# shicaiwei123/ICCV2025-GDL

Measured on AMD Instinct MI355X. Metric: audio-visual samples/sec, CREMA-D DGL train step (whole job), higher is better.
Workload: dtype bf16; 1 GPU; CREMA-D DGL (main_dgl.py, ConcatFusion_DGL) ResNet18 a+v, spec 1x257x188 + frames 3x3x224x224, alpha=4, SGD lr 2e-3 mom .9 wd 1e-4, clip 40; per_gpu_batch=64, global_batch=64, parallelism=dp1, buckets=none

## Files before the change

iccv2025-gdl_amd/csrc/conv_wgrad.hip:

```cpp
#include <stdlib.h>

#include "common.h"
#include "gather.h"
#include "prof.h"

#include <hip/hip_ext.h>

namespace gdl {

struct WgradArgs {
    const void* dy;
    const void* x;
    float* partial;
    const GatherEntry* table;
    int C, K, RS, M;
    int nsplit, chunk;
    int tiles_k, tiles_c;
    unsigned dy_bytes, x_bytes;
    int delta[9];
    int split;
    int delta_hi[9];
#ifdef GDL_TIMING
    unsigned long long* dbg;
#endif
// ... 142 lines not shown
#ifdef GDL_TIMING
    unsigned long long t_entry = __builtin_amdgcn_s_memtime(), t_wait = 0, t_comp = 0, t_issue = 0, t_a, t_b;
#endif
    if (nst > 0) load_stage(0);
#ifdef GDL_TIMING
    unsigned long long t_first = __builtin_amdgcn_s_memtime();
#endif
    for (int st = 0; st < nst; ++st) {
        const int buf = st & 1;
#ifdef GDL_TIMING
        t_a = __builtin_amdgcn_s_memtime();
#endif
        asm volatile("s_waitcnt vmcnt(0)" ::: "memory");
        __builtin_amdgcn_s_barrier();
        asm volatile("" ::: "memory");
#ifdef GDL_TIMING
        t_b = __builtin_amdgcn_s_memtime();
        t_wait += t_b - t_a;
#endif
        if (st + 1 < nst) load_stage(buf ^ 1);
#ifdef GDL_TIMING
        t_a = __builtin_amdgcn_s_memtime();
        t_issue += t_a - t_b;
#endif
        const unsigned Ks = smem_base + buf * STAGE;
        const unsigned Cs = Ks + WG_BP * PK;
        if (sizeof(T) == 2) {
#pragma unroll
            for (int ks = 0; ks < WG_BP / 32; ++ks) {
                uint2 alo[FK], ahi[FK], blo[FC], bhi[FC];
#pragma unroll
                for (int h = 0; h < 2; ++h) {
                    const int row = ks * 32 + g * 8 + h * 4 + (li >> 2);
#pragma unroll
                    for (int i = 0; i < FK; ++i) {
                        const int chb = (wk * WTK + i * 16 + (li & 3) * 4) * 2;
                        const int addr = row * PK + ((((chb >> 5) ^ wg_swz<PK>(row)) << 5) | (chb & 31));
                        if (h == 0)
                            alo[i] = lds_tr16_asm(Ks + addr);
                        else
                            ahi[i] = lds_tr16_asm(Ks + addr);
                    }
#pragma unroll
                    for (int jj = 0; jj < FC; ++jj) {
                        const int chb = (wc * WTC + jj * 16 + (li & 3) * 4) * 2;
                        const int addr = row * PC + ((((chb >> 5) ^ wg_swz<PC>(row)) << 5) | (chb & 31));
                        if (h == 0)
                            blo[jj] = lds_tr16_asm(Cs + addr);
                        else
                            bhi[jj] = lds_tr16_asm(Cs + addr);
                    }
                }
                wg_lds_wait();
#pragma unroll
                for (int i = 0; i < FK; ++i) {
                    const uint4 fa = make_uint4(alo[i].x, alo[i].y, ahi[i].x, ahi[i].y);
#pragma unroll
                    for (int jj = 0; jj < FC; ++jj) {
                        const uint4 fb = make_uint4(blo[jj].x, blo[jj].y, bhi[jj].x, bhi[jj].y);
                        acc[i][jj] = __builtin_amdgcn_mfma_f32_16x16x32_bf16(__builtin_bit_cast(bf16x8_t, fa),
                                                                           __builtin_bit_cast(bf16x8_t, fb), acc[i][jj], 0,
                                                                           0, 0);
                    }
                }
            }
        } else {
#pragma unroll 4
            for (int ks = 0; ks < WG_BP / 4; ++ks) {
                const int row = ks * 4 + g;
                float fa[FK], fb[FC];
#pragma unroll
                for (int i = 0; i < FK; ++i) {
                    const int chb = (wk * WTK + i * 16 + li) * 4;
                    fa[i] = lds_read_f32_asm(Ks + row * PK + ((((chb >> 5) ^ wg_swz<PK>(row)) << 5) | (chb & 31)));
                }
#pragma unroll
                for (int jj = 0; jj < FC; ++jj) {
                    const int chb = (wc * WTC + jj * 16 + li) * 4;
                    fb[jj] = lds_read_f32_asm(Cs + row * PC + ((((chb >> 5) ^ wg_swz<PC>(row)) << 5) | (chb & 31)));
                }
                wg_lds_wait();
#pragma unroll
                for (int i = 0; i < FK; ++i)
#pragma unroll
                    for (int jj = 0; jj < FC; ++jj)
                        acc[i][jj] = __builtin_amdgcn_mfma_f32_16x16x4f32(fa[i], fb[jj], acc[i][jj], 0, 0, 0);
            }
        }
    }
#ifdef GDL_TIMING
    unsigned long long t_loop_end = __builtin_amdgcn_s_memtime();
    t_comp = (t_loop_end - t_first) - t_wait - t_issue;
#endif
    float* part = a.partial + (size_t)slice * a.K * RS * a.C;
#pragma unroll
    for (int i = 0; i < FK; ++i)
#pragma unroll
        for (int jj = 0; jj < FC; ++jj) {
            const int c = c0 + wc * WTC + jj * 16 + li;
#pragma unroll
            for (int e = 0; e < 4; ++e) {
                const int k = k0 + wk * WTK + i * 16 + g * 4 + e;
                part[((size_t)k * RS + tap) * a.C + c] = acc[i][jj][e];
            }
        }
#ifdef GDL_TIMING
    if (a.dbg && tid == 0) {
        unsigned long long* d = a.dbg + (size_t)blockIdx.x * 8;
        d[0] = t_entry;
        d[1] = t_first - t_entry;
        d[2] = t_wait;
        d[3] = t_issue;
        d[4] = t_comp;
        d[5] = __builtin_amdgcn_s_memtime() - t_loop_end;
        d[6] = nst;
    }
#endif
}

template <int LANES>
__global__ __launch_bounds__(256) void wgrad_reduce_kernel(const float* __restrict__ partial, float* __restrict__ out,
                                                           int nsplit, int K, int RS, int C, int Cout) {
    constexpr int OUTS = 256 / LANES;
    __shared__ float red[LANES][OUTS];
    const size_t total = (size_t)K * RS * C;
    const int o = threadIdx.x % OUTS, l = threadIdx.x / OUTS;
    const size_t i = blockIdx.x * (size_t)OUTS + o;
    float s = 0.f;
    if (i < total)
        for (int sp = l; sp < nsplit; sp += LANES) s += partial[(size_t)sp * total + i];
    if (LANES > 1) {
        red[l][o] = s;
        __syncthreads();
        if (l == 0) {
            s = red[0][o];
#pragma unroll
            for (int j = 1; j < LANES; ++j) s += red[j][o];
        }
    }
    if (l == 0 && i < total) {
        const int c = (int)(i % C);
        const size_t t = i / C;
        const int rs = (int)(t % RS);
        const int k = (int)(t / RS);
        if (c < Cout) out[((size_t)k * Cout + c) * RS + rs] = s;
    }
}

bool conv_wgrad9_enabled();
bool conv_wgrad9_ok(int dtype, int W, int C, int K, int R, int S, int stride, int pad);
size_t conv_wgrad9_ws_bytes(int M, int C, int K);
int conv_wgrad9(const void* dy, const void* x, float* dw, const void* table, int N, int H, int W, int C, int K, void* ws,
                size_t ws_bytes, hipStream_t st);

struct WgradPlan {
    int tk, tc, nsplit, chunk;
};

static WgradPlan plan_wgrad(int M, int C, int K, int RS, bool gemm = false) {
    WgradPlan p;
    p.tk = (K % 128 == 0) ? 128 : 64;
    p.tc = (C % 128 == 0) ? 128 : 64;
    const int tiles = (K / p.tk) * (C / p.tc) * RS;
    static int forced = -1;
    if (forced < 0) {
        const char* e = tune_env("GDL_WGRAD_BLOCKS");
        forced = e ? atoi(e) : 0;
    }
    static int forced_gemm = -1;
    if (forced_gemm < 0) {
        const char* e = tune_env("GDL_WGRAD_GEMM_BLOCKS");
        forced_gemm = e ? atoi(e) : 0;
    }
    const int target = (gemm && forced_gemm > 0) ? forced_gemm : forced > 0 ? forced : (gemm ? 416 : 128);
    int ns = (target + tiles - 1) / tiles;
    const int max_ns = (M + 2 * WG_BP - 1) / (2 * WG_BP);
    if (ns > max_ns) ns = max_ns;
    if (ns < 1) ns = 1;
    int chunk = (M + ns - 1) / ns;
    chunk = (chunk + WG_BP - 1) / WG_BP * WG_BP;
    p.nsplit = (M + chunk - 1) / chunk;
    p.chunk = chunk;
    return p;
}

size_t conv_wgrad_ws_bytes(int M, int C, int K, int RS) {
    const WgradPlan p = plan_wgrad(M, C, K, RS, RS == 1);
    size_t b = (size_t)p.nsplit * K * RS * C * sizeof(float);
    if (RS == 9 && conv_wgrad9_enabled()) {
        const size_t b9 = conv_wgrad9_ws_bytes(M, C, K);
        if (b9 > b) b = b9;
    }
    return b;
}

template <typename T, int TK, int TC>
static int launch_wg(WgradArgs& a, hipStream_t st) {
    constexpr int BYTES = 2 * WG_BP * (TK + TC) * (int)sizeof(T);
    auto kfn = conv_wgrad_kernel<T, TK, TC>;
    static DevOnce attr_set;
    if (!attr_set) {
        hipError_t e = hipFuncSetAttribute((const void*)kfn, hipFuncAttributeMaxDynamicSharedMemorySize, BYTES);
        if (e != hipSuccess) return check_hip(e, "hipFuncSetAttribute(conv_wgrad)");
        attr_set = true;
    }
    const int per_slice = a.RS * a.tiles_k * a.tiles_c;
    const int grid = xcd_grid(a.nsplit * per_slice);
    static char pname[96] = "";
    if (!pname[0]) snprintf(pname, sizeof(pname), "gdl::conv_wgrad_kernel<%s, %d, %d>", prof_tname<T>(), TK, TC);
    ProfScope prof(pname, PROF_MFMA, st, 2.0 * (double)a.M * a.K * a.C * a.RS, true,
                   (double)a.dy_bytes + (double)a.x_bytes + 4.0 * (double)a.K * a.C * a.RS);
    hipExtLaunchKernelGGL(kfn, dim3(grid), dim3(256), BYTES, st, prof.e0(), prof.e1(), 0, a);
    GDL_CHECK_LAUNCH("conv_wgrad_kernel");
    return GDL_OK;
}

int conv_wgrad(int dtype, const void* dy, const void* x, float* dw, const void* table, int N, int H, int W, int C, int K,
               int R, int S, int stride, int pad, int Cout, void* ws, size_t ws_bytes, hipStream_t st) {
    GDL_REQUIRE(dtype == GDL_BF16 || dtype == GDL_F32, "wgrad: bad dtype %d", dtype);
    GDL_REQUIRE(table, "wgrad: gather table is null (build it with gdl_conv_build_table)");
    GDL_REQUIRE(C % 64 == 0 && K % 64 == 0, "wgrad: C=%d K=%d must be multiples of 64", C, K);
    if (Cout == C && conv_wgrad9_ok(dtype, W, C, K, R, S, stride, pad))
        return conv_wgrad9(dy, x, dw, table, N, H, W, C, K, ws, ws_bytes, st);
    GatherGeom g;
    int rc = gather_geom(GATHER_FWD, dtype, N, H, W, C, K, R, S, stride, pad, &g);
    if (rc) return rc;
    const int esz = dtype == GDL_BF16 ? 2 : 4;
    WgradArgs a{};
#ifdef GDL_TIMING
    a.dbg = g_timing_buf;
#endif
    a.dy = dy;
    a.x = x;
    a.table = (const GatherEntry*)table;
    a.C = C;
    a.K = K;
    a.RS = R * S;
    a.M = g.rows;
    for (int t = 0; t < 9; ++t) a.delta[t] = g.delta[t];
    GDL_REQUIRE(a.M < (1 << 24), "wgrad: M exceeds 2^24");
    GDL_REQUIRE((size_t)a.M * K * esz < (1UL << 31), "wgrad: dy exceeds 2 GiB");
    a.dy_bytes = (unsigned)((size_t)a.M * K * esz);
    a.x_bytes = (unsigned)((size_t)N * H * W * C * esz);
    const WgradPlan p = plan_wgrad(a.M, C, K, R * S, R == 1 && S == 1 && stride == 1);
    a.nsplit = p.nsplit;
    a.chunk = p.chunk;
    a.tiles_k = K / p.tk;
    a.tiles_c = C / p.tc;
    const size_t need = (size_t)p.nsplit * K * R * S * C * sizeof(float);
    if (ws_bytes < need || !ws) {
        set_error("wgrad: workspace %zu < %zu bytes", ws_bytes, need);
        return GDL_ERR_WORKSPACE;
    }
    a.partial = (float*)ws;
    if (dtype == GDL_BF16) {
        if (p.tk == 128 && p.tc == 128)
            rc = launch_wg<bf16, 128, 128>(a, st);
        else if (p.tk == 128)
            rc = launch_wg<bf16, 128, 64>(a, st);
        else if (p.tc == 128)
            rc = launch_wg<bf16, 64, 128>(a, st);
        else
            rc = launch_wg<bf16, 64, 64>(a, st);
    } else {
        if (p.tk == 128 && p.tc == 128)
            rc = launch_wg<float, 128, 128>(a, st);
        else if (p.tk == 128)
            rc = launch_wg<float, 128, 64>(a, st);
        else if (p.tc == 128)
            rc = launch_wg<float, 64, 128>(a, st);
        else
            rc = launch_wg<float, 64, 64>(a, st);
    }
    if (rc) return rc;
    const size_t total = (size_t)K * R * S * C;
#ifdef GDL_EXPERIMENT
    if (experiment_mask2() & 1) return GDL_OK;
#endif
    ProfScope prof(p.nsplit >= 64 ? "gdl::wgrad_reduce_kernel<16>" : (p.nsplit > 8 ? "gdl::wgrad_reduce_kernel<4>" : "gdl::wgrad_reduce_kernel<1>"),
                   PROF_HBM, st, (double)total * 4.0 * (p.nsplit + 1));
    if (p.nsplit >= 64)
        hipLaunchKernelGGL(wgrad_reduce_kernel<16>, dim3((unsigned)((total + 15) / 16)), dim3(256), 0, st, a.partial, dw,
                           p.nsplit, K, R * S, C, Cout);
    else if (p.nsplit > 8)
        hipLaunchKernelGGL(wgrad_reduce_kernel<4>, dim3((unsigned)((total + 63) / 64)), dim3(256), 0, st, a.partial, dw,
                           p.nsplit, K, R * S, C, Cout);
    else
        hipLaunchKernelGGL(wgrad_reduce_kernel<1>, dim3((unsigned)((total + 255) / 256)), dim3(256), 0, st, a.partial, dw,
                           p.nsplit, K, R * S, C, Cout);
    GDL_CHECK_LAUNCH("wgrad_reduce_kernel");
    return GDL_OK;
}

__global__ __launch_bounds__(256) void stem_wgrad_reduce_kernel(const float* __restrict__ partial, float* __restrict__ out,
                                                                int nsplit, int Cin) {
    __shared__ float4 red[16][16];
    constexpr int TILE4 = 64 * 4 * 64 / 4;
    const int o = threadIdx.x & 15, l = threadIdx.x >> 4;
    const int idx4 = blockIdx.x * 16 + o;
    const float4* p = (const float4*)partial + idx4;
    float4 s = make_float4(0.f, 0.f, 0.f, 0.f);
    int sp = l;
    for (; sp + 48 < nsplit; sp += 64) {
        const float4 v0 = p[(size_t)sp * TILE4], v1 = p[(size_t)(sp + 16) * TILE4];
        const float4 v2 = p[(size_t)(sp + 32) * TILE4], v3 = p[(size_t)(sp + 48) * TILE4];
        s.x += v0.x, s.y += v0.y, s.z += v0.z, s.w += v0.w;
        s.x += v1.x, s.y += v1.y, s.z += v1.z, s.w += v1.w;
        s.x += v2.x, s.y += v2.y, s.z += v2.z, s.w += v2.w;
        s.x += v3.x, s.y += v3.y, s.z += v3.z, s.w += v3.w;
    }
    for (; sp < nsplit; sp += 16) {
        const float4 v0 = p[(size_t)sp * TILE4];
        s.x += v0.x, s.y += v0.y, s.z += v0.z, s.w += v0.w;
    }
    red[l][o] = s;
    __syncthreads();
    if (l != 0) return;
#pragma unroll
    for (int jj = 1; jj < 16; ++jj) {
        const float4 v = red[jj][o];
        s.x += v.x, s.y += v.y, s.z += v.z, s.w += v.w;
    }
    const int q = idx4 & 15, tap = (idx4 >> 4) & 3, k = idx4 >> 6;
    const int r = 2 * tap + (q >> 3), px = q & 7;
    if (r < 7 && px < 7) {
        const float v[4] = {s.x, s.y, s.z, s.w};
        for (int c = 0; c < Cin; ++c) out[((k * Cin + c) * 7 + r) * 7 + px] = v[c];
    }
}

struct StemRowsArgs {
    const void* dy;
    const void* xp;
    float* partial;
    int P, Q, Hp, Wp, nseg;
    int stages, chunk, nsplit;
    unsigned dy_bytes, x_bytes;
};
constexpr int SR_PITCH = 1088, SR_XBYTES = 9 * 1024, SR_STAGE = 8192 + SR_XBYTES;
template <int OFF>
__device__ __forceinline__ uint2 sr_tr(unsigned addr) {
    uint2 v;
    asm volatile("ds_read_b64_tr_b16 %0, %1 offset:%2" : "=v"(v) : "v"(addr), "n"(OFF));
    return v;
}
template <int N>
__device__ __forceinline__ void sr_wait() {
    __builtin_amdgcn_sched_barrier(0);
    asm volatile("s_waitcnt lgkmcnt(%0)" ::"n"(N) : "memory");
    __builtin_amdgcn_sched_barrier(0);
}
__global__ __launch_bounds__(256) void stem_wgrad_rows_kernel(StemRowsArgs a) {
    extern __shared__ __attribute__((aligned(16))) unsigned char smem[];
    const int tid = threadIdx.x, lane = tid & 63, wave = __builtin_amdgcn_readfirstlane(tid >> 6);
    const int g = lane >> 4, li = lane & 15;
    const int slice = blockIdx.x;
    const int s_begin = slice * a.chunk, s_end = min(a.stages, s_begin + a.chunk);
    const int nst = s_end - s_begin;
    const unsigned smem_base = (unsigned)(uintptr_t)(const __attribute__((address_space(3))) unsigned char*)smem;
    const __amdgpu_buffer_rsrc_t rdy = __builtin_amdgcn_make_buffer_rsrc((void*)a.dy, 0, a.dy_bytes, 0x00020000);
    const __amdgpu_buffer_rsrc_t rx = __builtin_amdgcn_make_buffer_rsrc((void*)a.xp, 0, a.x_bytes, 0x00020000);

    const int prow = lane >> 3, pch = lane & 7;
    int dy_rel[2];
#pragma unroll
    for (int i = 0; i < 2; ++i) {
        const int row = (wave + 4 * i) * 8 + prow;
        const int ch = (((pch >> 1) ^ wg_swz<128>(row)) << 1) | (pch & 1);
        dy_rel[i] = row * 128 + ch * 16;
    }
    int x_rel[3];
#pragma unroll
    for (int i = 0; i < 3; ++i) {
        const int p = wave + 4 * i, off = 1024 * p + 16 * lane;
        const int row = off / SR_PITCH, col = off % SR_PITCH;
        x_rel[i] = (p < 9 && row < 8 && col < 1072) ? row * a.Wp * 8 + col : -1;
// ... 528 lines not shown
```

iccv2025-gdl_amd/csrc/conv_wgrad9.hip:

```cpp
#include <stdlib.h>

#include "common.h"
#include "gather.h"
#include "prof.h"

#include <hip/hip_ext.h>

namespace gdl {

struct Wgrad9Args {
    const void* dy;
    const void* x;
    float* partial;
    const GatherEntry* table;
    int C, K, M, W;
    int nsplit, chunk;
    int tiles_k, tiles_c;
    int slab_rows;
    unsigned dy_bytes, x_bytes;
#ifdef GDL_TIMING
    unsigned long long* dbg;
#endif
};
#ifdef GDL_TIMING
extern unsigned long long* g_timing_buf;
#endif

constexpr int W9_BP = 64;

__device__ __forceinline__ void w9_dma16(__amdgpu_buffer_rsrc_t rsrc, unsigned char* lds_base, int voffset) {
#if defined(__HIP_DEVICE_COMPILE__)
    __builtin_amdgcn_raw_ptr_buffer_load_lds(rsrc, (__attribute__((address_space(3))) void*)lds_base, 16, voffset, 0, 0, 0);
#else
    (void)rsrc;
    (void)lds_base;
    (void)voffset;
#endif
}
__device__ __forceinline__ void w9_dma4(__amdgpu_buffer_rsrc_t rsrc, unsigned char* lds_base, int voffset) {
#if defined(__HIP_DEVICE_COMPILE__)
    __builtin_amdgcn_raw_ptr_buffer_load_lds(rsrc, (__attribute__((address_space(3))) void*)lds_base, 4, voffset, 0, 0, 0);
#else
    (void)rsrc;
    (void)lds_base;
    (void)voffset;
#endif
}
template <int OFF>
__device__ __forceinline__ unsigned w9_lds32(unsigned addr) {
    unsigned v;
    asm volatile("ds_read_b32 %0, %1 offset:%2" : "=v"(v) : "v"(addr), "n"(OFF));
    return v;
}
template <int OFF>
__device__ __forceinline__ uint2 w9_tr(unsigned addr) {
    uint2 v;
    asm volatile("ds_read_b64_tr_b16 %0, %1 offset:%2" : "=v"(v) : "v"(addr), "n"(OFF));
    return v;
}
template <int N>
__device__ __forceinline__ void w9_wait() {
    __builtin_amdgcn_sched_barrier(0);
    asm volatile("s_waitcnt lgkmcnt(%0)" ::"n"(N) : "memory");
    __builtin_amdgcn_sched_barrier(0);
}
__device__ __forceinline__ int w9_swz(int row) { return ((row >> 1) & 1) | (((row >> 3) & 1) << 1); }

template <int RING>
__global__ __launch_bounds__(256, 2) void conv_wgrad9_kernel(Wgrad9Args a) {
    extern __shared__ __attribute__((aligned(16))) unsigned char smem[];
    const int tid = threadIdx.x, lane = tid & 63, wave = __builtin_amdgcn_readfirstlane(tid >> 6);
    const int g = lane >> 4, li = lane & 15;

    const int per_slice = a.tiles_k * a.tiles_c;
    const int L = xcd_linear(a.nsplit * per_slice);
    if (L < 0) return;
    const int slice = L / per_slice, rem = L - slice * per_slice;
    const int kt = rem % a.tiles_k, ct = rem / a.tiles_k;
    const int k0 = kt * 64, c0 = ct * 64;
    const int m_begin = slice * a.chunk;
    const int m_end = min(a.M, m_begin + a.chunk);
    const int nst = (m_end - m_begin + W9_BP - 1) / W9_BP;

    const int nins = (a.slab_rows + 7) >> 3;
    constexpr int W9_RING = RING * 32768;
    const int STAGE = RING ? W9_BP * 128 : W9_BP * 128 + nins * 1024;
    const int DY0 = RING ? W9_RING + 4096 : 0;
    const int ZOFF = RING ? DY0 + 2 * STAGE : 2 * STAGE;
    const unsigned smem_base = (unsigned)(uintptr_t)(const __attribute__((address_space(3))) unsigned char*)smem;
    if (RING && (smem_base & (unsigned)(W9_RING > 0 ? W9_RING - 1 : 0)) != 0) __builtin_trap();
    unsigned char* zero_p = smem + ZOFF;
    unsigned char* mask_st = zero_p + 1024;
    const unsigned zrow = smem_base + ZOFF;
    const int ringT = ((2 * a.W + 2 + 63) >> 6) << 6;

    const __amdgpu_buffer_rsrc_t rdy = __builtin_amdgcn_make_buffer_rsrc((void*)a.dy, 0, a.dy_bytes, 0x00020000);
    const __amdgpu_buffer_rsrc_t rx = __builtin_amdgcn_make_buffer_rsrc((void*)a.x, 0, a.x_bytes, 0x00020000);
    const __amdgpu_buffer_rsrc_t rtab =
        __builtin_amdgcn_make_buffer_rsrc((void*)a.table, 0, (unsigned)a.M * (unsigned)sizeof(GatherEntry), 0x00020000);
    if (wave == 0) w9_dma16(rx, zero_p, (int)0x80000000);

    const int prow = lane >> 3, pch = lane & 7;
    int ld_m = m_begin;
    int ld_s = 0;
    auto load_stage = [&](int buf) {
        unsigned char* Ks = smem + DY0 + buf * STAGE;
        unsigned char* Xs = Ks + W9_BP * 128;
        const int blk = (ld_s + (ringT >> 6)) & (RING ? RING * 4 - 1 : 3);
        const int nx = !RING ? nins : (ld_s == 0 ? (ringT >> 3) + 8 : (blk == 0 ? 12 : 8));
        const int np = 8 + nx + 1;
        for (int p = wave; p < np; p += 4) {
            if (p < 8) {
                const int row = p * 8 + prow, m = ld_m + row;
                const int ch = (((pch >> 1) ^ w9_swz(row)) << 1) | (pch & 1);
                w9_dma16(rdy, Ks + p * 1024, m < m_end ? m * (a.K * 2) + k0 * 2 + ch * 16 : (int)0x80000000);
            } else if (RING && p < 8 + nx) {
                int jj = p - 8;
                int pix, dst;
                if (ld_s == 0) {
                    pix = m_begin - (a.W + 1) - (ringT - 2 * a.W - 2) + jj * 8 + prow;
                    dst = jj * 1024;
                } else {
                    const bool mir = jj >= 8;
                    if (mir) jj -= 8;
                    pix = ld_m + (a.W + 1) + jj * 8 + prow;
                    dst = mir ? W9_RING + jj * 1024 : blk * 8192 + jj * 1024;
                }
                const int sr = jj * 8 + prow;
                const int ch = (((pch >> 1) ^ w9_swz(sr)) << 1) | (pch & 1);
                w9_dma16(rx, smem + dst, (unsigned)pix < (unsigned)a.M ? pix * (a.C * 2) + c0 * 2 + ch * 16 : (int)0x80000000);
            } else if (!RING && p < 8 + nins) {
                const int jj = p - 8, sr = jj * 8 + prow;
                const int pix = ld_m - (a.W + 1) + sr;
                const bool ok = sr < a.slab_rows && (unsigned)pix < (unsigned)a.M;
                const int ch = (((pch >> 1) ^ w9_swz(sr)) << 1) | (pch & 1);
                w9_dma16(rx, Xs + jj * 1024, ok ? pix * (a.C * 2) + c0 * 2 + ch * 16 : (int)0x80000000);
            } else {
                const int m = ld_m + lane;
                w9_dma4(rtab, mask_st + buf * 256, m < m_end ? m * (int)sizeof(GatherEntry) + 4 : (int)0x80000000);
            }
        }
        ld_m += W9_BP;
        ld_s += 1;
    };

    const int K2 = a.K * 2, C2 = a.C * 2;
    int dyb, xb, mb;
    {
        const int row = wave * 8 + prow;
        const int ch = (((pch >> 1) ^ w9_swz(row)) << 1) | (pch & 1);
        dyb = (m_begin + W9_BP + row) * K2 + k0 * 2 + ch * 16;
        xb = (m_begin + W9_BP + (RING ? a.W + 1 : -(a.W + 1)) + row) * C2 + c0 * 2 + ch * 16;
        mb = (m_begin + W9_BP + lane) * (int)sizeof(GatherEntry) + 4;
    }
    auto load_fast = [&](int buf) {
        unsigned char* Ks = smem + DY0 + buf * STAGE;
        w9_dma16(rdy, Ks + wave * 1024, dyb);
        w9_dma16(rdy, Ks + (wave + 4) * 1024, dyb + 32 * K2);
        if (RING) {
            const int rb = (ld_s + (ringT >> 6)) & (RING ? RING * 4 - 1 : 3);
            unsigned char* dst = smem + rb * 8192;
            w9_dma16(rx, dst + wave * 1024, xb);
            w9_dma16(rx, dst + (wave + 4) * 1024, xb + 32 * C2);
            if (rb == 0) w9_dma16(rx, smem + W9_RING + wave * 1024, xb);
        } else {
            unsigned char* Xs = Ks + W9_BP * 128;
            int o = 0;
            for (int jj = wave; jj < nins; jj += 4, o += 32 * C2) w9_dma16(rx, Xs + jj * 1024, xb + o);
        }
        if (wave == 0) w9_dma4(rtab, mask_st + buf * 256, mb);
        dyb += W9_BP * K2;
        xb += W9_BP * C2;
        mb += W9_BP * (int)sizeof(GatherEntry);
        ld_m += W9_BP;
        ld_s += 1;
    };

    const int lrow = g * 8 + (li >> 2);
    unsigned aaddr[4][2];
#pragma unroll
    for (int h = 0; h < 2; ++h) {
        const int row = lrow + h * 4;
#pragma unroll
        for (int i = 0; i < 4; ++i) aaddr[i][h] = smem_base + DY0 + row * 128 + ((i ^ w9_swz(row)) << 5) + (li & 3) * 8;
    }
    unsigned baddr[9][2];
#pragma unroll
    for (int t = 0; t < 9; ++t) {
        const int sh = (t / 3 - 1) * a.W + (t % 3 - 1);
#pragma unroll
        for (int h = 0; h < 2; ++h) {
            const int sr = lrow + h * 4 + (a.W + 1) + sh + (RING ? ringT - 2 * a.W - 2 : 0);
            baddr[t][h] = smem_base + (RING ? 0 : W9_BP * 128) + sr * 128 + ((wave ^ w9_swz(sr)) << 5) + (li & 3) * 8;
        }
    }
    const unsigned zaddr = zrow + (li & 3) * 8;
    const unsigned maddr = zrow + 1024 + lrow * 4;

    f32x4_t acc[9][4];
#pragma unroll
    for (int t = 0; t < 9; ++t)
#pragma unroll
        for (int i = 0; i < 4; ++i) acc[t][i] = f32x4_t{0.f, 0.f, 0.f, 0.f};

#ifdef GDL_TIMING
    unsigned long long t_entry = __builtin_amdgcn_s_memtime(), t_wait = 0, t_issue = 0, t_a, t_b;
#endif
    if (nst > 0) load_stage(0);
#ifdef GDL_TIMING
    unsigned long long t_first = __builtin_amdgcn_s_memtime();
#endif
    for (int st = 0; st < nst; ++st) {
#ifdef GDL_TIMING
        t_a = __builtin_amdgcn_s_memtime();
#endif
        asm volatile("s_waitcnt vmcnt(0)" ::: "memory");
        __builtin_amdgcn_s_barrier();
        asm volatile("" ::: "memory");
#ifdef GDL_TIMING
// ... 138 lines not shown
        const int tap = (int)(r % 9);
        r /= 9;
        const int wave = (int)(r & 3);
        const int tile = (int)(r >> 2);
        const int kt = tile % tiles_k, ct = tile / tiles_k;
        const int k = kt * 64 + i * 16 + (lane >> 4) * 4, c = ct * 64 + wave * 16 + (lane & 15);
        float* dst = out + ((size_t)k * C + c) * 9 + tap;
        const size_t kstride = (size_t)C * 9;
        dst[0] = s.x;
        dst[kstride] = s.y;
        dst[2 * kstride] = s.z;
        dst[3 * kstride] = s.w;
    }
}

__global__ __launch_bounds__(256) void wgrad9_reduce_rows_kernel(const float4* __restrict__ partial, float* __restrict__ out,
                                                                 int nsplit, int K, int C, int tiles_k, int tiles_c) {
    __shared__ float patch[16][16 * 9];
    const size_t total4 = (size_t)K * C * 9 / 4;
    const int lane = threadIdx.x & 63, w4 = threadIdx.x >> 6;
    const int grp = blockIdx.x;
    const int i = grp & 3, wave = (grp >> 2) & 3, tile = grp >> 4;
    const int kk = (lane >> 4) * 4, cc = lane & 15;
    for (int tap = w4; tap < 9; tap += 4) {
        const size_t idx = (((size_t)(tile * 4 + wave) * 9 + tap) * 4 + i) * 64 + lane;
        float4 s = partial[idx];
        for (int sp = 1; sp < nsplit; ++sp) {
            const float4 v = partial[(size_t)sp * total4 + idx];
            s.x += v.x, s.y += v.y, s.z += v.z, s.w += v.w;
        }
        patch[kk + 0][cc * 9 + tap] = s.x;
        patch[kk + 1][cc * 9 + tap] = s.y;
        patch[kk + 2][cc * 9 + tap] = s.z;
        patch[kk + 3][cc * 9 + tap] = s.w;
    }
    __syncthreads();
    const int kt = tile % tiles_k, ct = tile / tiles_k;
    const int k0 = kt * 64 + i * 16, c0 = ct * 64 + wave * 16;
    for (int t = threadIdx.x; t < 16 * 36; t += 256) {
        const int r = t / 36, q = t - r * 36;
        *(float4*)(out + ((size_t)(k0 + r) * C + c0) * 9 + 4 * q) = *(const float4*)&patch[r][4 * q];
    }
}

struct W9Plan {
    int nsplit, chunk;
};
static W9Plan plan_w9(int M, int C, int K) {
    const int tiles = (K / 64) * (C / 64);
    constexpr int target = 256;
    static int min_st = -1;
    if (min_st < 0) {
        const char* e = tune_env("GDL_WGRAD9_MINST");
        min_st = e ? atoi(e) : 56;
    }
    int ns = (target + tiles - 1) / tiles;
    const int max_ns = (M + min_st * W9_BP - 1) / (min_st * W9_BP);
    if (ns > max_ns) ns = max_ns;
    if (ns < 1) ns = 1;
    int chunk = (M + ns - 1) / ns;
    chunk = (chunk + W9_BP - 1) / W9_BP * W9_BP;
    W9Plan p;
    p.nsplit = (M + chunk - 1) / chunk;
    p.chunk = chunk;
    return p;
}

bool conv_wgrad9_enabled() {
    static int v = -1;
    if (v < 0) {
        const char* e = tune_env("GDL_WGRAD9");
        v = e ? atoi(e) : 1;
    }
    return v != 0;
}

size_t conv_wgrad9_ws_bytes(int M, int C, int K) {
    const W9Plan p = plan_w9(M, C, K);
    return (size_t)p.nsplit * K * 9 * C * sizeof(float);
}

static int w9_ring(int W) {
    static int v = -1;
    if (v < 0) {
        const char* e = tune_env("GDL_WGRAD9_RING");
        v = e ? atoi(e) : 1;
    }
    if (v == 0 || W < 24) return 0;
    if (2 * W + 2 <= 128) return 1;
    const int rows = W9_BP + 2 * W + 2;
    const size_t plain = 2 * (size_t)(W9_BP * 128 + ((rows + 7) / 8) * 1024) + 1024 + 512;
    return (plain > 80 * 1024 && 2 * W + 2 <= 384) ? 2 : 0;
}
static size_t w9_lds_bytes(int W) {
    const int ring = w9_ring(W);
    if (ring) return (size_t)ring * 32768 + 4096 + 2 * W9_BP * 128 + 1024 + 512;
    const int rows = W9_BP + 2 * W + 2;
    return 2 * (size_t)(W9_BP * 128 + ((rows + 7) / 8) * 1024) + 1024 + 512;
}

bool conv_wgrad9_ok(int dtype, int W, int C, int K, int R, int S, int stride, int pad) {
    return conv_wgrad9_enabled() && dtype == GDL_BF16 && R == 3 && S == 3 && stride == 1 && pad == 1 && C % 64 == 0 &&
           K % 64 == 0 && w9_lds_bytes(W) <= 96 * 1024;
}

int conv_wgrad9(const void* dy, const void* x, float* dw, const void* table, int N, int H, int W, int C, int K, void* ws,
                size_t ws_bytes, hipStream_t st) {
    Wgrad9Args a{};
#ifdef GDL_TIMING
    a.dbg = g_timing_buf;
#endif
    a.dy = dy;
    a.x = x;
    a.table = (const GatherEntry*)table;
    a.C = C;
    a.K = K;
    a.M = N * H * W;
    a.W = W;
    GDL_REQUIRE(a.M < (1 << 24), "wgrad: M exceeds 2^24");
    GDL_REQUIRE((size_t)a.M * K * 2 < (1UL << 31) && (size_t)a.M * C * 2 < (1UL << 31), "wgrad: tensor exceeds 2 GiB");
    a.dy_bytes = (unsigned)((size_t)a.M * K * 2);
    a.x_bytes = (unsigned)((size_t)a.M * C * 2);
    const W9Plan p = plan_w9(a.M, C, K);
    a.nsplit = p.nsplit;
    a.chunk = p.chunk;
    a.tiles_k = K / 64;
    a.tiles_c = C / 64;
    a.slab_rows = W9_BP + 2 * W + 2;
    const size_t need = (size_t)p.nsplit * K * 9 * C * sizeof(float);
    if (ws_bytes < need || !ws) {
        set_error("wgrad: workspace %zu < %zu bytes", ws_bytes, need);
        return GDL_ERR_WORKSPACE;
    }
    a.partial = (float*)ws;
    const size_t lds = w9_lds_bytes(W);
    const int ring = w9_ring(W);
    using KernT = void (*)(Wgrad9Args);
    static const KernT kerns[3] = {conv_wgrad9_kernel<0>, conv_wgrad9_kernel<1>, conv_wgrad9_kernel<2>};
    const KernT kern = kerns[ring];
    static DevOnce attr_set[3];
    if (!attr_set[ring]) {
        hipError_t e = hipFuncSetAttribute((const void*)kern, hipFuncAttributeMaxDynamicSharedMemorySize, 96 * 1024);
        if (e != hipSuccess) return check_hip(e, "hipFuncSetAttribute(conv_wgrad9)");
        attr_set[ring] = true;
    }
    const int per_slice = a.tiles_k * a.tiles_c;
    const int grid = xcd_grid(a.nsplit * per_slice);
    {
        ProfScope prof("gdl::conv_wgrad9_kernel", PROF_MFMA, st, 2.0 * (double)a.M * K * C * 9, true,
                       2.0 * (double)a.M * (K + C) + 4.0 * (double)K * C * 9);
        hipExtLaunchKernelGGL(kern, dim3(grid), dim3(256), lds, st, prof.e0(), prof.e1(), 0, a);
        GDL_CHECK_LAUNCH("conv_wgrad9_kernel");
    }
    const size_t total4 = (size_t)K * C * 9 / 4;
#ifdef GDL_EXPERIMENT
    if (experiment_mask2() & 1) return GDL_OK;
#endif
    ProfScope prof("gdl::wgrad9_reduce_kernel", PROF_HBM, st, (double)total4 * 16.0 * (p.nsplit + 1));
    if (p.nsplit <= 4)
        hipLaunchKernelGGL(wgrad9_reduce_rows_kernel, dim3((unsigned)(a.tiles_k * a.tiles_c * 16)), dim3(256), 0, st,
                           (const float4*)a.partial, dw, p.nsplit, K, C, a.tiles_k, a.tiles_c);
    else
        hipLaunchKernelGGL(wgrad9_reduce_kernel<16>, dim3((unsigned)((total4 + 15) / 16)), dim3(256), 0, st,
                           (const float4*)a.partial, dw, p.nsplit, K, C, a.tiles_k, a.tiles_c);
    GDL_CHECK_LAUNCH("wgrad9_reduce_kernel");
    return GDL_OK;
}

}
```

Measured before the change: 13070 samples/s.

## Add specialized stride-2 3x3 weight-gradient kernel with parity-plane LDS rings

Adds a dedicated bf16 weight-gradient kernel for 3x3 stride-2 pad-1 convolutions. It loads four input parity planes into LDS ring buffers via buffer-to-LDS DMA and reuses each staged row across all nine taps with masked LDS reads feeding MFMA. This replaces the generic gathered wgrad path, which is meant to cut redundant global gathers. The kernel runs at one block per CU with a large LDS footprint, and it reuses the existing split-K fold reduction, now factored into a shared helper.

Measured after the change: 13120 samples/s (median of 6 runs). About the same (+0.4%).

```diff
diff --git a/iccv2025-gdl_amd/csrc/conv_wgrad.hip b/iccv2025-gdl_amd/csrc/conv_wgrad.hip
--- a/iccv2025-gdl_amd/csrc/conv_wgrad.hip
+++ b/iccv2025-gdl_amd/csrc/conv_wgrad.hip
@@ -318,6 +318,11 @@
 size_t conv_wgrad9_ws_bytes(int M, int C, int K);
 int conv_wgrad9(const void* dy, const void* x, float* dw, const void* table, int N, int H, int W, int C, int K, void* ws,
                 size_t ws_bytes, hipStream_t st);
+bool conv_wgrad9s2_enabled();
+bool conv_wgrad9s2_ok(int dtype, int W, int C, int K, int R, int S, int stride, int pad);
+size_t conv_wgrad9s2_ws_bytes(int M, int C, int K);
+int conv_wgrad9s2(const void* dy, const void* x, float* dw, const void* table, int N, int H, int W, int C, int K, void* ws,
+                  size_t ws_bytes, hipStream_t st);
 
 struct WgradPlan {
     int tk, tc, nsplit, chunk;
@@ -357,6 +362,10 @@
         const size_t b9 = conv_wgrad9_ws_bytes(M, C, K);
         if (b9 > b) b = b9;
     }
+    if (RS == 9 && conv_wgrad9s2_enabled()) {
+        const size_t b9 = conv_wgrad9s2_ws_bytes(M, C, K);
+        if (b9 > b) b = b9;
+    }
     return b;
 }
 
@@ -388,6 +397,8 @@
     GDL_REQUIRE(C % 64 == 0 && K % 64 == 0, "wgrad: C=%d K=%d must be multiples of 64", C, K);
     if (Cout == C && conv_wgrad9_ok(dtype, W, C, K, R, S, stride, pad))
         return conv_wgrad9(dy, x, dw, table, N, H, W, C, K, ws, ws_bytes, st);
+    if (Cout == C && conv_wgrad9s2_ok(dtype, W, C, K, R, S, stride, pad))
+        return conv_wgrad9s2(dy, x, dw, table, N, H, W, C, K, ws, ws_bytes, st);
     GatherGeom g;
     int rc = gather_geom(GATHER_FWD, dtype, N, H, W, C, K, R, S, stride, pad, &g);
     if (rc) return rc;
diff --git a/iccv2025-gdl_amd/csrc/conv_wgrad9.hip b/iccv2025-gdl_amd/csrc/conv_wgrad9.hip
--- a/iccv2025-gdl_amd/csrc/conv_wgrad9.hip
+++ b/iccv2025-gdl_amd/csrc/conv_wgrad9.hip
@@ -3,6 +3,7 @@
 #include "common.h"
 #include "gather.h"
 #include "prof.h"
+#include "wgrad9_dev.h"
 
 #include <hip/hip_ext.h>
 
@@ -26,45 +27,6 @@
 extern unsigned long long* g_timing_buf;
 #endif
 
-constexpr int W9_BP = 64;
-
-__device__ __forceinline__ void w9_dma16(__amdgpu_buffer_rsrc_t rsrc, unsigned char* lds_base, int voffset) {
-#if defined(__HIP_DEVICE_COMPILE__)
-    __builtin_amdgcn_raw_ptr_buffer_load_lds(rsrc, (__attribute__((address_space(3))) void*)lds_base, 16, voffset, 0, 0, 0);
-#else
-    (void)rsrc;
-    (void)lds_base;
-    (void)voffset;
-#endif
-}
-__device__ __forceinline__ void w9_dma4(__amdgpu_buffer_rsrc_t rsrc, unsigned char* lds_base, int voffset) {
-#if defined(__HIP_DEVICE_COMPILE__)
-    __builtin_amdgcn_raw_ptr_buffer_load_lds(rsrc, (__attribute__((address_space(3))) void*)lds_base, 4, voffset, 0, 0, 0);
-#else
-    (void)rsrc;
-    (void)lds_base;
-    (void)voffset;
-#endif
-}
-template <int OFF>
-__device__ __forceinline__ unsigned w9_lds32(unsigned addr) {
-    unsigned v;
-    asm volatile("ds_read_b32 %0, %1 offset:%2" : "=v"(v) : "v"(addr), "n"(OFF));
-    return v;
-}
-template <int OFF>
-__device__ __forceinline__ uint2 w9_tr(unsigned addr) {
-    uint2 v;
-    asm volatile("ds_read_b64_tr_b16 %0, %1 offset:%2" : "=v"(v) : "v"(addr), "n"(OFF));
-    return v;
-}
-template <int N>
-__device__ __forceinline__ void w9_wait() {
-    __builtin_amdgcn_sched_barrier(0);
-    asm volatile("s_waitcnt lgkmcnt(%0)" ::"n"(N) : "memory");
-    __builtin_amdgcn_sched_barrier(0);
-}
-__device__ __forceinline__ int w9_swz(int row) { return ((row >> 1) & 1) | (((row >> 3) & 1) << 1); }
 
 template <int RING>
 __global__ __launch_bounds__(256, 2) void conv_wgrad9_kernel(Wgrad9Args a) {
@@ -509,17 +471,22 @@
         hipExtLaunchKernelGGL(kern, dim3(grid), dim3(256), lds, st, prof.e0(), prof.e1(), 0, a);
         GDL_CHECK_LAUNCH("conv_wgrad9_kernel");
     }
+    return wgrad9_fold(a.partial, dw, p.nsplit, K, C, st);
+}
+
+int wgrad9_fold(const float* partial, float* dw, int nsplit, int K, int C, hipStream_t st) {
+    const int tiles_k = K / 64, tiles_c = C / 64;
     const size_t total4 = (size_t)K * C * 9 / 4;
 #ifdef GDL_EXPERIMENT
     if (experiment_mask2() & 1) return GDL_OK;
 #endif
-    ProfScope prof("gdl::wgrad9_reduce_kernel", PROF_HBM, st, (double)total4 * 16.0 * (p.nsplit + 1));
-    if (p.nsplit <= 4)
-        hipLaunchKernelGGL(wgrad9_reduce_rows_kernel, dim3((unsigned)(a.tiles_k * a.tiles_c * 16)), dim3(256), 0, st,
-                           (const float4*)a.partial, dw, p.nsplit, K, C, a.tiles_k, a.tiles_c);
+    ProfScope prof("gdl::wgrad9_reduce_kernel", PROF_HBM, st, (double)total4 * 16.0 * (nsplit + 1));
+    if (nsplit <= 4)
+        hipLaunchKernelGGL(wgrad9_reduce_rows_kernel, dim3((unsigned)(tiles_k * tiles_c * 16)), dim3(256), 0, st,
+                           (const float4*)partial, dw, nsplit, K, C, tiles_k, tiles_c);
     else
         hipLaunchKernelGGL(wgrad9_reduce_kernel<16>, dim3((unsigned)((total4 + 15) / 16)), dim3(256), 0, st,
-                           (const float4*)a.partial, dw, p.nsplit, K, C, a.tiles_k, a.tiles_c);
+                           (const float4*)partial, dw, nsplit, K, C, tiles_k, tiles_c);
     GDL_CHECK_LAUNCH("wgrad9_reduce_kernel");
     return GDL_OK;
 }
diff --git a/iccv2025-gdl_amd/csrc/conv_wgrad9s2.hip b/iccv2025-gdl_amd/csrc/conv_wgrad9s2.hip
--- /dev/null
+++ b/iccv2025-gdl_amd/csrc/conv_wgrad9s2.hip
@@ -0,0 +1,353 @@
+#include <stdlib.h>
+
+#include "common.h"
+#include "gather.h"
+#include "prof.h"
+#include "wgrad9_dev.h"
+
+#include <hip/hip_ext.h>
+
+namespace gdl {
+
+struct Wgrad9s2Args {
+    const void* dy;
+    const void* x;
+    float* partial;
+    const GatherEntry* table;
+    int C, K, M, Q;
+    int nsplit, chunk;
+    int tiles_k, tiles_c;
+    int pdelta[4];
+    unsigned dy_bytes, x_bytes;
+};
+
+constexpr int S2_BLK = W9_BP * 128;
+constexpr int S2_RING = 3 * S2_BLK;
+constexpr int S2_DY0 = 4 * S2_RING;
+constexpr int S2_ZOFF = S2_DY0 + 2 * S2_BLK;
+constexpr int S2_TOFF = S2_ZOFF + 1024;
+constexpr int S2_LDS = S2_TOFF + 4 * 512;
+
+template <int OFF>
+__device__ __forceinline__ uint2 s2_lds64(unsigned addr) {
+    uint2 v;
+    asm volatile("ds_read_b64 %0, %1 offset:%2" : "=v"(v) : "v"(addr), "n"(OFF));
+    return v;
+}
+
+__global__ __launch_bounds__(256, 1) void conv_wgrad9s2_kernel(Wgrad9s2Args a) {
+    extern __shared__ __attribute__((aligned(16))) unsigned char smem[];
+    const int tid = threadIdx.x, lane = tid & 63, wave = __builtin_amdgcn_readfirstlane(tid >> 6);
+    const int g = lane >> 4, li = lane & 15;
+
+    const int per_slice = a.tiles_k * a.tiles_c;
+    const int L = xcd_linear(a.nsplit * per_slice);
+    if (L < 0) return;
+    const int slice = L / per_slice, rem = L - slice * per_slice;
+    const int kt = rem % a.tiles_k, ct = rem / a.tiles_k;
+    const int k0 = kt * 64, c0 = ct * 64;
+    const int m_begin = slice * a.chunk;
+    const int m_end = min(a.M, m_begin + a.chunk);
+    const int nst = (m_end - m_begin + W9_BP - 1) / W9_BP;
+
+    const unsigned smem_base = (unsigned)(uintptr_t)(const __attribute__((address_space(3))) unsigned char*)smem;
+    if (smem_base != 0) __builtin_trap();
+
+    const __amdgpu_buffer_rsrc_t rdy = __builtin_amdgcn_make_buffer_rsrc((void*)a.dy, 0, a.dy_bytes, 0x00020000);
+    const __amdgpu_buffer_rsrc_t rx = __builtin_amdgcn_make_buffer_rsrc((void*)a.x, 0, a.x_bytes, 0x00020000);
+    const __amdgpu_buffer_rsrc_t rtab =
+        __builtin_amdgcn_make_buffer_rsrc((void*)a.table, 0, (unsigned)a.M * (unsigned)sizeof(GatherEntry), 0x00020000);
+    constexpr int OOB = (int)0x80000000;
+    if (wave == 0) w9_dma16(rx, smem + S2_ZOFF, OOB);
+
+    const int prow = lane >> 3, pch = lane & 7;
+    const int row0 = wave * 8 + prow;
+    const int K2 = a.K * 2;
+    int pofs[4];
+    int dyb;
+    {
+        const int ch = (((pch >> 1) ^ w9_swz(row0)) << 1) | (pch & 1);
+#pragma unroll
+        for (int pl = 0; pl < 4; ++pl) pofs[pl] = a.pdelta[pl] + c0 * 2 + ch * 16;
+        dyb = (m_begin + row0) * K2 + k0 * 2 + ch * 16;
+    }
+    auto plane_pieces = [&](int blk, uint2 e0, uint2 e1) __attribute__((always_inline)) {
+#pragma unroll
+        for (int pl = 0; pl < 4; ++pl) {
+            const int bit = pl == 0 ? 8 : pl == 1 ? 5 : pl == 2 ? 7 : 4;
+            unsigned char* dst = smem + pl * S2_RING + blk * S2_BLK;
+            w9_dma16(rx, dst + wave * 1024, ((e0.y >> bit) & 1u) ? (int)e0.x + pofs[pl] : OOB);
+            w9_dma16(rx, dst + (wave + 4) * 1024, ((e1.y >> bit) & 1u) ? (int)e1.x + pofs[pl] : OOB);
+        }
+    };
+    int ld_m = m_begin;
+    auto dy_pieces = [&](int buf) __attribute__((always_inline)) {
+        unsigned char* Ks = smem + S2_DY0 + buf * S2_BLK;
+        w9_dma16(rdy, Ks + wave * 1024, ld_m + row0 < m_end ? dyb : OOB);
+        w9_dma16(rdy, Ks + (wave + 4) * 1024, ld_m + row0 + 32 < m_end ? dyb + 32 * K2 : OOB);
+        dyb += W9_BP * K2;
+        ld_m += W9_BP;
+    };
+    auto table_pieces = [&](int s) __attribute__((always_inline)) {
+        if (wave < 2) {
+            const int h = wave * 256;
+            w9_dma4(rtab, smem + S2_TOFF + (s & 3) * 512 + h, (m_begin + s * W9_BP) * (int)sizeof(GatherEntry) + h + lane * 4);
+        }
+    };
+
+    auto gent = [&](int m) {
+        uint2 e = make_uint2(0u, 0u);
+        if ((unsigned)m < (unsigned)a.M) e = *(const uint2*)(a.table + m);
+        return e;
+    };
+    uint2 ent0 = make_uint2(0u, 0u), ent1 = ent0;
+    if (nst > 0) {
+        plane_pieces(0, gent(m_begin - 64 + row0), gent(m_begin - 32 + row0));
+        plane_pieces(1, gent(m_begin + row0), gent(m_begin + 32 + row0));
+        dy_pieces(0);
+        table_pieces(0);
+        table_pieces(1);
+        table_pieces(2);
+        ent0 = gent(m_begin + 64 + row0);
+        ent1 = gent(m_begin + 96 + row0);
+        asm volatile("" : "+v"(ent0.x), "+v"(ent0.y), "+v"(ent1.x), "+v"(ent1.y));
+    }
+    int ldblk = 2;
+
+    const int lrow = g * 8 + (li >> 2);
+    unsigned aaddr[4][2];
+#pragma unroll
+    for (int h = 0; h < 2; ++h) {
+        const int row = lrow + h * 4;
+#pragma unroll
+        for (int i = 0; i < 4; ++i) aaddr[i][h] = S2_DY0 + row * 128 + ((i ^ w9_swz(row)) << 5) + (li & 3) * 8;
+    }
+    unsigned raddr[4][2][2], a00[2][2];
+#pragma unroll
+    for (int j = 0; j < 4; ++j) {
+        const int sh = j == 0 ? 0 : j == 1 ? -1 : j == 2 ? -a.Q : -a.Q - 1;
+#pragma unroll
+        for (int ks = 0; ks < 2; ++ks)
+#pragma unroll
+            for (int h = 0; h < 2; ++h) {
+                const int rr = 64 + ks * 32 + lrow + h * 4 + sh;
+                raddr[j][ks][h] = rr * 128 + ((wave ^ w9_swz(rr)) << 5) + (li & 3) * 8;
+            }
+    }
+#pragma unroll
+    for (int ks = 0; ks < 2; ++ks)
+#pragma unroll
+        for (int h = 0; h < 2; ++h) a00[ks][h] = raddr[0][ks][h] + 3 * S2_RING;
+    unsigned zb[3];
+#pragma unroll
+    for (int pl = 0; pl < 3; ++pl) zb[pl] = S2_ZOFF - pl * S2_RING + (li & 3) * 8;
+    const unsigned maddr = S2_TOFF + lrow * 8 + 4;
+    const unsigned eaddr = S2_TOFF + row0 * 8;
+    auto ring_next = [](unsigned r) __attribute__((always_inline)) {
+        const unsigned n = r + (unsigned)S2_BLK;
+        return min(n, n - (unsigned)S2_RING);
+    };
+
+    f32x4_t acc[9][4];
+#pragma unroll
+    for (int t = 0; t < 9; ++t)
+#pragma unroll
+        for (int i = 0; i < 4; ++i) acc[t][i] = f32x4_t{0.f, 0.f, 0.f, 0.f};
+
+    for (int st = 0; st < nst; ++st) {
+        asm volatile("s_waitcnt vmcnt(0)" ::: "memory");
+        __builtin_amdgcn_s_barrier();
+        asm volatile("" ::: "memory");
+        unsigned pmask[2][2];
+        uint2 af[2][4][2];
+        uint2 nent0, nent1;
+        {
+            const unsigned ma = maddr + (st & 3) * 512;
+            pmask[0][0] = w9_lds32<0>(ma);
+            pmask[0][1] = w9_lds32<32>(ma);
+            pmask[1][0] = w9_lds32<256>(ma);
+            pmask[1][1] = w9_lds32<288>(ma);
+#pragma unroll
+            for (int i = 0; i < 4; ++i)
+#pragma unroll
+                for (int h = 0; h < 2; ++h) af[0][i][h] = w9_tr<0>(aaddr[i][h]);
+            const unsigned ea = eaddr + ((st + 2) & 3) * 512;
+            nent0 = s2_lds64<0>(ea);
+            nent1 = s2_lds64<256>(ea);
+        }
+        if (st + 1 < nst) {
+            dy_pieces((st + 1) & 1);
+            plane_pieces(ldblk, ent0, ent1);
+            table_pieces(st + 3);
+            ldblk = ldblk == 2 ? 0 : ldblk + 1;
+        }
+        w9_wait<0>();
+        ent0 = nent0;
+        ent1 = nent1;
+        constexpr int S2_AHEAD = 3, S2_A1 = 4;
+        uint2 bf[S2_AHEAD + 1][2];
+        auto issue_b = [&](int u) __attribute__((always_inline)) {
+            const int ks = u / 9, t = u % 9;
+            const int j = t == 0 ? 3 : (t == 1 || t == 2) ? 2 : (t == 3 || t == 6) ? 1 : 0;
+            const int pl = (t == 1 || t == 7) ? 2 : (t == 3 || t == 5) ? 1 : t == 4 ? 3 : 0;
+            const bool masked = t < 4 || t == 6;
+#pragma unroll
+            for (int h = 0; h < 2; ++h) {
+                unsigned ad = pl == 3 ? a00[ks][h] : raddr[j][ks][h];
+                if (masked) {
+                    unsigned sel, r2;
+                    asm("v_bfe_i32 %0, %1, %2, 1" : "=v"(sel) : "v"(pmask[ks][h]), "n"(t));
+                    asm("v_bfi_b32 %0, %1, %2, %3" : "=v"(r2) : "v"(sel), "v"(ad), "v"(zb[pl]));
+                    ad = r2;
+                }
+                bf[u % (S2_AHEAD + 1)][h] = pl == 1 ? w9_tr<S2_RING>(ad) : pl == 2 ? w9_tr<2 * S2_RING>(ad) : w9_tr<0>(ad);
+            }
+            if (t == 0 || t == 2 || t == 6 || t == 8) {
+#pragma unroll
+                for (int h = 0; h < 2; ++h) raddr[j][ks][h] = ring_next(raddr[j][ks][h]);
+            }
+            if (t == 8) {
+#pragma unroll
+                for (int h = 0; h < 2; ++h) a00[ks][h] = raddr[0][ks][h] + 3 * S2_RING;
+            }
+        };
+#pragma unroll
+        for (int u = 0; u < S2_AHEAD; ++u) issue_b(u);
+#pragma unroll
+        for (int u = 0; u < 18; ++u) {
+            const int ks = u / 9, t = u % 9;
+            if (u + S2_AHEAD < 18) issue_b(u + S2_AHEAD);
+            if (u == S2_A1) {
+#pragma unroll
+                for (int i = 0; i < 4; ++i)
+#pragma unroll
+                    for (int h = 0; h < 2; ++h) af[1][i][h] = w9_tr<4096>(aaddr[i][h]);
+            }
+            const int nb = (18 - 1 - u < S2_AHEAD ? 18 - 1 - u : S2_AHEAD) * 2;
+            const bool a1_younger = u >= S2_A1 && u <= S2_A1 + S2_AHEAD && u < 9;
+            switch (nb + (a1_younger ? 8 : 0)) {
+                case 0: w9_wait<0>(); break;
+                case 2: w9_wait<2>(); break;
+                case 4: w9_wait<4>(); break;
+                case 6: w9_wait<6>(); break;
+                case 8: w9_wait<8>(); break;
+                case 10: w9_wait<10>(); break;
+                case 12: w9_wait<12>(); break;
+                default: w9_wait<14>(); break;
+            }
+            const uint2* b2 = bf[u % (S2_AHEAD + 1)];
+            const uint4 fb = make_uint4(b2[0].x, b2[0].y, b2[1].x, b2[1].y);
+#pragma unroll
+            for (int i = 0; i < 4; ++i) {
+                const uint4 fa = make_uint4(af[ks][i][0].x, af[ks][i][0].y, af[ks][i][1].x, af[ks][i][1].y);
+                acc[t][i] = __builtin_amdgcn_mfma_f32_16x16x32_bf16(__builtin_bit_cast(bf16x8_t, fa),
+                                                                   __builtin_bit_cast(bf16x8_t, fb), acc[t][i], 0, 0, 0);
+            }
+        }
+        const int dlt = (st & 1) ? -S2_BLK : S2_BLK;
+#pragma unroll
+        for (int i = 0; i < 4; ++i)
+#pragma unroll
+            for (int h = 0; h < 2; ++h) aaddr[i][h] += dlt;
+    }
+    float4* part = (float4*)a.partial + ((((size_t)slice * per_slice + rem) * 4 + wave) * 36) * 64;
+#pragma unroll
+    for (int t = 0; t < 9; ++t)
+#pragma unroll
+        for (int i = 0; i < 4; ++i)
+            part[(t * 4 + i) * 64 + lane] = make_float4(acc[t][i][0], acc[t][i][1], acc[t][i][2], acc[t][i][3]);
+}
+
+struct W9s2Plan {
+    int nsplit, chunk;
+};
+static W9s2Plan plan_w9s2(int M, int C, int K) {
+    const int tiles = (K / 64) * (C / 64);
+    constexpr int target = 256;
+    static int min_st = -1;
+    if (min_st < 0) {
+        const char* e = tune_env("GDL_WGRAD9S2_MINST");
+        min_st = e ? atoi(e) : 48;
+        if (min_st < 1) min_st = 1;
+    }
+    int ns = (target + tiles - 1) / tiles;
+    const int max_ns = (M + min_st * W9_BP - 1) / (min_st * W9_BP);
+    if (ns > max_ns) ns = max_ns;
+    if (ns < 1) ns = 1;
+    int chunk = (M + ns - 1) / ns;
+    chunk = (chunk + W9_BP - 1) / W9_BP * W9_BP;
+    W9s2Plan p;
+    p.nsplit = (M + chunk - 1) / chunk;
+    p.chunk = chunk;
+    return p;
+}
+
+bool conv_wgrad9s2_enabled() {
+    static int v = -1;
+    if (v < 0) {
+        const char* e = tune_env("GDL_WGRAD9S2");
+        v = e ? atoi(e) : 1;
+    }
+    return v != 0;
+}
+
+size_t conv_wgrad9s2_ws_bytes(int M, int C, int K) {
+    const W9s2Plan p = plan_w9s2(M, C, K);
+    return (size_t)p.nsplit * K * 9 * C * sizeof(float);
+}
+
+bool conv_wgrad9s2_ok(int dtype, int W, int C, int K, int R, int S, int stride, int pad) {
+    const int Q = (W - 1) / 2 + 1;
+    return conv_wgrad9s2_enabled() && dtype == GDL_BF16 && R == 3 && S == 3 && stride == 2 && pad == 1 && C % 64 == 0 &&
+           K % 64 == 0 && Q + 1 <= W9_BP;
+}
+
+int conv_wgrad9s2(const void* dy, const void* x, float* dw, const void* table, int N, int H, int W, int C, int K, void* ws,
+                  size_t ws_bytes, hipStream_t st) {
+    GatherGeom g;
+    int rc = gather_geom(GATHER_FWD, GDL_BF16, N, H, W, C, K, 3, 3, 2, 1, &g);
+    if (rc) return rc;
+    Wgrad9s2Args a{};
+    a.dy = dy;
+    a.x = x;
+    a.table = (const GatherEntry*)table;
+    a.C = C;
+    a.K = K;
+    a.M = g.rows;
+    a.Q = (W - 1) / 2 + 1;
+    a.pdelta[0] = g.delta[8];
+    a.pdelta[1] = g.delta[5];
+    a.pdelta[2] = g.delta[7];
+    a.pdelta[3] = g.delta[4];
+    GDL_REQUIRE(a.M < (1 << 24), "wgrad: M exceeds 2^24");
+    GDL_REQUIRE((size_t)a.M * K * 2 < (1UL << 31), "wgrad: dy exceeds 2 GiB");
+    a.dy_bytes = (unsigned)((size_t)a.M * K * 2);
+    a.x_bytes = (unsigned)((size_t)N * H * W * C * 2);
+    const W9s2Plan p = plan_w9s2(a.M, C, K);
+    a.nsplit = p.nsplit;
+    a.chunk = p.chunk;
+    a.tiles_k = K / 64;
+    a.tiles_c = C / 64;
+    const size_t need = (size_t)p.nsplit * K * 9 * C * sizeof(float);
+    if (ws_bytes < need || !ws) {
+        set_error("wgrad: workspace %zu < %zu bytes", ws_bytes, need);
+        return GDL_ERR_WORKSPACE;
+    }
+    a.partial = (float*)ws;
+    static DevOnce attr_set;
+    if (!attr_set) {
+        hipError_t e = hipFuncSetAttribute((const void*)conv_wgrad9s2_kernel, hipFuncAttributeMaxDynamicSharedMemorySize, S2_LDS);
+        if (e != hipSuccess) return check_hip(e, "hipFuncSetAttribute(conv_wgrad9s2)");
+        attr_set = true;
+    }
+    const int grid = xcd_grid(a.nsplit * a.tiles_k * a.tiles_c);
+    {
+        ProfScope prof("gdl::conv_wgrad9s2_kernel", PROF_MFMA, st, 2.0 * (double)a.M * K * C * 9, true,
+                       (double)a.dy_bytes + (double)a.x_bytes + 4.0 * (double)K * C * 9);
+        hipExtLaunchKernelGGL(conv_wgrad9s2_kernel, dim3(grid), dim3(256), S2_LDS, st, prof.e0(), prof.e1(), 0, a);
+        GDL_CHECK_LAUNCH("conv_wgrad9s2_kernel");
+    }
+    return wgrad9_fold(a.partial, dw, p.nsplit, K, C, st);
+}
+
+}
diff --git a/iccv2025-gdl_amd/csrc/wgrad9_dev.h b/iccv2025-gdl_amd/csrc/wgrad9_dev.h
--- /dev/null
+++ b/iccv2025-gdl_amd/csrc/wgrad9_dev.h
@@ -0,0 +1,48 @@
+#pragma once
+#include "common.h"
+
+namespace gdl {
+
+constexpr int W9_BP = 64;
+
+__device__ __forceinline__ void w9_dma16(__amdgpu_buffer_rsrc_t rsrc, unsigned char* lds_base, int voffset) {
+#if defined(__HIP_DEVICE_COMPILE__)
+    __builtin_amdgcn_raw_ptr_buffer_load_lds(rsrc, (__attribute__((address_space(3))) void*)lds_base, 16, voffset, 0, 0, 0);
+#else
+    (void)rsrc;
+    (void)lds_base;
+    (void)voffset;
+#endif
+}
+__device__ __forceinline__ void w9_dma4(__amdgpu_buffer_rsrc_t rsrc, unsigned char* lds_base, int voffset) {
+#if defined(__HIP_DEVICE_COMPILE__)
+    __builtin_amdgcn_raw_ptr_buffer_load_lds(rsrc, (__attribute__((address_space(3))) void*)lds_base, 4, voffset, 0, 0, 0);
+#else
+    (void)rsrc;
+    (void)lds_base;
+    (void)voffset;
+#endif
+}
+template <int OFF>
+__device__ __forceinline__ unsigned w9_lds32(unsigned addr) {
+    unsigned v;
+    asm volatile("ds_read_b32 %0, %1 offset:%2" : "=v"(v) : "v"(addr), "n"(OFF));
+    return v;
+}
+template <int OFF>
+__device__ __forceinline__ uint2 w9_tr(unsigned addr) {
+    uint2 v;
+    asm volatile("ds_read_b64_tr_b16 %0, %1 offset:%2" : "=v"(v) : "v"(addr), "n"(OFF));
+    return v;
+}
+template <int N>
+__device__ __forceinline__ void w9_wait() {
+    __builtin_amdgcn_sched_barrier(0);
+    asm volatile("s_waitcnt lgkmcnt(%0)" ::"n"(N) : "memory");
+    __builtin_amdgcn_sched_barrier(0);
+}
+__device__ __forceinline__ int w9_swz(int row) { return ((row >> 1) & 1) | (((row >> 3) & 1) << 1); }
+
+int wgrad9_fold(const float* partial, float* dw, int nsplit, int K, int C, hipStream_t st);
+
+}
```
